# Distributed-Deep-Learning/ps

Measured on AMD Instinct MI355X. Metric: samples/sec (whole node) ResNet-50 sync-BSP at 1/2/4/8 MI355X workers, higher is better.
Workload: dtype bf16; 1 GPU; model=ResNet-50, global_batch=1024, image_size=224, parallelism=ps-bsp-colocated-dp1, optimizer=momentum@lr:0.1@momentum:0.9@wd:5e-05@nesterov:0.0@, staleness=0, fused_bn=True, ranks_per_device=1, compute_priority=high, side_stream=True, streams_per_rank=3, data_plane=local

## Files before the change

csrc/bindings.cpp:

```cpp
#include <torch/extension.h>
#include <c10/hip/HIPStream.h>
#include <c10/core/DeviceGuard.h>

#include "psamd_launch.h"

#include <atomic>
#include <map>
#include <mutex>
#include <string>

namespace {

std::atomic<bool> g_route_on{false};
std::mutex g_route_mu;
std::map<std::string, int64_t>& routes() {
  static std::map<std::string, int64_t> r;
  return r;
}
void route(const std::string& name) {
  if (!g_route_on.load(std::memory_order_relaxed)) return;
  std::lock_guard<std::mutex> g(g_route_mu);
  routes()[name] += 1;
}
std::map<std::string, int64_t> route_log(bool enable, bool reset) {
// ... 1693 lines not shown
                              want_mask ? mb.data_ptr<uint8_t>() : nullptr, R, static_cast<int>(C),
                              static_cast<int>(act), cur_stream(x));
  return {y, mb};
}

void weight_prep(Tensor jobs, int64_t max_blocks) {
  check_gpu(jobs, "jobs");
  TORCH_CHECK(jobs.scalar_type() == torch::kInt64 && jobs.dim() == 2 && jobs.size(1) == 4 && jobs.is_contiguous(),
              "jobs: int64 [J, 4]");
  static_assert(sizeof(void*) == 8, "64-bit pointers");
  const c10::DeviceGuard guard(jobs.device());
  TORCH_CHECK(max_blocks > 0 && max_blocks < (1 << 20), "max_blocks");
  psamd::launch_weight_prep(jobs.data_ptr(), static_cast<int>(jobs.size(0)), static_cast<int>(max_blocks),
                            cur_stream(jobs));
}

std::vector<Tensor> bn_bwd_coef(Tensor part, c10::optional<Tensor> gamma, Tensor mean, Tensor invstd, int64_t R) {
  check_part_slabs(part);
  const int64_t C = part.size(2);
  TORCH_CHECK(C % 8 == 0, "C % 8");
  const c10::DeviceGuard guard(part.device());
  auto fopt = part.options();
  auto dg = torch::empty({C}, fopt), db = torch::empty({C}, fopt), coef = torch::empty({3 * C}, fopt);
  const Tensor fp = fold_partials(part, cur_stream(part));
  const int64_t Gf = fp.size(1);
  psamd::launch_bn_bwd_partials(fp.data_ptr<float>(), fp.data_ptr<float>() + fp.stride(0), static_cast<int>(Gf), nullptr,
                                nullptr, f32_opt(gamma, C, "gamma"), f32_opt(mean, C, "mean"), f32_opt(invstd, C, "invstd"),
                                dg.data_ptr<float>(), db.data_ptr<float>(), coef.data_ptr<float>(), nullptr, R,
                                static_cast<int>(C), cur_stream(part));
  return {dg, db, coef};
}

std::vector<Tensor> bn_bwd_partials(Tensor g, Tensor x, Tensor part, c10::optional<Tensor> gamma, Tensor mean,
                                    Tensor invstd) {
  check_rows(g, "g");
  check_rows(x, "x");
  TORCH_CHECK(x.dim() == 2 && g.sizes() == x.sizes() && x.size(1) % 8 == 0, "g/x [R, C], C % 8");
  const int64_t R = x.size(0), C = x.size(1);
  check_part_slabs(part);
  TORCH_CHECK(part.size(2) == C, "part [2, G, C]");
  const c10::DeviceGuard guard(x.device());
  auto fopt = x.options().dtype(torch::kFloat32);
  auto dx = torch::empty_like(x);
  auto dg = torch::empty({C}, fopt), db = torch::empty({C}, fopt), coef = torch::empty({3 * C}, fopt);
  const Tensor fp = fold_partials(part, cur_stream(x));
  const int64_t Gf = fp.size(1);
  psamd::launch_bn_bwd_partials(fp.data_ptr<float>(), fp.data_ptr<float>() + fp.stride(0), static_cast<int>(Gf), u16(g), u16(x),
                                f32_opt(gamma, C, "gamma"), f32_opt(mean, C, "mean"), f32_opt(invstd, C, "invstd"),
                                dg.data_ptr<float>(), db.data_ptr<float>(), coef.data_ptr<float>(), u16m(dx), R,
                                static_cast<int>(C), cur_stream(x));
  return {dx, dg, db};
}

}

void register_async_ps(pybind11::module& m);
void register_plane(pybind11::module& m);
void register_async_rows(pybind11::module& m);

PYBIND11_MODULE(TORCH_EXTENSION_NAME, m) {
  m.doc() = "ps_amd HIP kernels for MI355X (gfx950)";
  register_async_ps(m);
  register_plane(m);
  register_async_rows(m);
  m.def("conv_gemm", &conv_gemm, py::arg("a"), py::arg("b"), py::arg("geo"), py::arg("pro") = py::none(),
        py::arg("epi") = 0, py::arg("aux") = py::none(), py::arg("kshift") = py::none(), py::arg("mc") = py::none(),
        py::arg("mean") = py::none(), py::arg("invstd") = py::none(), py::arg("bits") = py::none(),
        py::arg("aux2") = py::none(), py::arg("bits2") = py::none(), py::arg("a2") = py::none(),
        py::arg("bwd") = py::none(), py::arg("aux3") = py::none(), py::arg("mean2") = py::none(),
        py::arg("invstd2") = py::none(), py::arg("pro2") = py::none(), py::arg("aout") = py::none(),
        py::arg("abits") = py::none(), py::arg("tbuf") = py::none());
  m.def("route_log", &route_log, py::arg("enable") = true, py::arg("reset") = true);
  m.def("linear_wgrad_db", &linear_wgrad_db);
  m.def("bn_bwd_coef", &bn_bwd_coef);
  m.def("weight_prep", &weight_prep, py::arg("jobs"), py::arg("max_blocks") = 1024);
  m.def("conv_dgrad_s2", &conv_dgrad_s2, py::arg("dz"), py::arg("wph"), py::arg("H"), py::arg("W"),
        py::arg("epi") = 0, py::arg("z") = py::none(), py::arg("mc") = py::none(), py::arg("mean") = py::none(),
        py::arg("invstd") = py::none());
  m.def("conv_wgrad", &conv_wgrad, py::arg("dz"), py::arg("x"), py::arg("geo"), py::arg("pro") = py::none());
  m.def("conv_wgrad_patch_ok", &conv_wgrad_patch_ok, py::arg("geo"), py::arg("images"), py::arg("N"), py::arg("C"));
  {
    py::dict epi;
    epi["STORE"] = static_cast<int>(psamd::kEpiStore);
    epi["STATS"] = static_cast<int>(psamd::kEpiStats);
    epi["ADD"] = static_cast<int>(psamd::kEpiAdd);
    epi["MASK_SUMS"] = static_cast<int>(psamd::kEpiMaskSums);
    epi["ADD_S2"] = static_cast<int>(psamd::kEpiAddS2);
    epi["ADD_MASKED"] = static_cast<int>(psamd::kEpiAddMasked);
    epi["FOLD_ADD_MASKED"] = static_cast<int>(psamd::kEpiFoldAddMasked);
    epi["FOLD_ADD"] = static_cast<int>(psamd::kEpiFoldAdd);
    epi["FOLD_ADD_S2"] = static_cast<int>(psamd::kEpiFoldAddS2);
    epi["FOLD_ADD_MASKED_DS"] = static_cast<int>(psamd::kEpiFoldAddMaskedDs);
    m.attr("EPI") = epi;
  }
  m.attr("kTwosrcGldsMinNk") = psamd::kTwosrcGldsMinNk;
  m.def("conv_gemm_plan", &conv_gemm_plan, py::arg("M"), py::arg("N"), py::arg("C"), py::arg("geo"),
        py::arg("pro") = false, py::arg("epi") = 0, py::arg("src2") = 0);
  m.def("conv11_bwd_fused", &conv11_bwd_fused, py::arg("g"), py::arg("z3"), py::arg("cbwd"), py::arg("wt"), py::arg("z2"),
        py::arg("cf2") = py::none(), py::arg("mean2") = py::none(), py::arg("invstd2") = py::none());
  m.def("conv11_bwd_fused_supported", &conv11_bwd_fused_supported, py::arg("ci"), py::arg("co"),
        py::arg("plain") = false);
  m.def("bn_apply_coef", &bn_apply_coef, py::arg("x"), py::arg("coef"), py::arg("res") = py::none(),
        py::arg("rcoef") = py::none(), py::arg("act") = 1, py::arg("want_mask") = false);
  m.def("bn_bwd_partials", &bn_bwd_partials);
  m.def("fused_opt", &fused_opt);
  m.def("sparse_opt", &sparse_opt, py::arg("kind"), py::arg("table"), py::arg("st0"), py::arg("st1"),
        py::arg("rows"), py::arg("grad"), py::arg("rowwise"), py::arg("skip_zero"), py::arg("lr"), py::arg("beta1"),
        py::arg("beta2"), py::arg("eps"), py::arg("wd"), py::arg("momentum"), py::arg("dampening"),
        py::arg("nesterov"), py::arg("adamw"), py::arg("bc1"), py::arg("bc2"), py::arg("l1"), py::arg("l2"),
        py::arg("fbeta"), py::arg("ftrl_mode"), py::arg("gscale"), py::arg("perm") = py::none(), py::arg("ncount") = py::none());
  m.def("sumsq", &sumsq);
  m.def("clip_factor", &clip_factor);
  m.def("cast_", &cast_);
  m.def("axpy_", &axpy_);
  m.def("reduce_n", &reduce_n);
  m.def("lerp", &lerp);
  m.def("onebit_pack", &onebit_pack, py::arg("g"), py::arg("err"), py::arg("words"), py::arg("scales"),
        py::arg("mom") = py::none(), py::arg("beta1") = 0.0);
  m.def("onebit_momentum", &onebit_momentum);
  m.def("onebit_unpack_reduce", &onebit_unpack_reduce);
  m.def("gather_rows", &gather_rows);
  m.def("segment_reduce_rows", &segment_reduce_rows);
  m.def("bag_pool_fwd", &bag_pool_fwd);
  m.def("bag_pool_bwd", &bag_pool_bwd);
  m.def("scatter_add_rows", &scatter_add_rows);
  m.def("embedding_bag_fwd", &embedding_bag_fwd);
  m.def("sparse_lr_fwd", &sparse_lr_fwd);
  m.def("lazy_init_rows", &lazy_init_rows, py::arg("table"), py::arg("rows"), py::arg("flags"), py::arg("seed"),
        py::arg("row_base"), py::arg("lo"), py::arg("hi"), py::arg("keys") = py::none());
  m.def("hash_slots", &hash_slots);
  m.def("rehash_rows", &rehash_rows);
  m.def("unique_runs", &unique_runs);
  m.def("softmax_temp_fwd", &softmax_temp_fwd);
  m.def("softmax_temp_bwd", &softmax_temp_bwd);
  m.def("softmax_xent", &softmax_xent);
  m.def("bce", &bce);
  m.def("maxpool2d_fwd", &maxpool2d_fwd);
  m.def("maxpool2d_bwd", &maxpool2d_bwd);
  m.def("im2col", &im2col);
  m.def("col2im", &col2im);
  m.def("dropout", &dropout);
  m.def("uniform_init", &uniform_init);
  m.def("gemm_nt", &gemm_nt);
  m.def("fc_bwd", &fc_bwd, py::arg("dy"), py::arg("y"), py::arg("x"), py::arg("w"), py::arg("dw") = py::none(),
        py::arg("db") = py::none(), py::arg("dx") = py::none(), py::arg("act") = 0);
  m.def("fc_fwd_f32", &fc_fwd_f32);
  m.def("act_bwd", &act_bwd);
  m.def("bn_act_fwd", &bn_act_fwd);
  m.def("bn_stats", &bn_stats);
  m.def("maxpool_nhwc_fwd", &maxpool_nhwc_fwd);
  m.def("stem_conv_fwd", &stem_conv_fwd, py::arg("x"), py::arg("wp"), py::arg("kshift") = py::none());
  m.def("bn_finalize_sums", &bn_finalize_sums);
  m.def("stem_conv_wrw", &stem_conv_wrw);
  m.def("stem_bwd_fused", &stem_bwd_fused);
  m.def("dlrm_interact_fwd", &dlrm_interact_fwd);
  m.def("rmsnorm_fwd", &rmsnorm_fwd);
  m.def("rmsnorm_bwd", &rmsnorm_bwd);
// ... 27 lines not shown
```

csrc/include/psamd_launch.h:

```cpp
#pragma once
#include <hip/hip_runtime.h>
#include <stdint.h>

#include <stdexcept>
#include <string>

namespace psamd {

struct FusedOptArgs {
  int kind;
  float* w;
  float* st0;
  float* st1;
  const void* g;
  int g_bf16;
  void* wout;
  int wout_bf16;
  int64_t n;
  float lr, beta1, beta2, eps, wd, momentum, dampening;
  int nesterov, adamw;
  float bc1, bc2;
  float l1, l2, fbeta;
  int ftrl_mode;
  float gscale;
// ... 388 lines not shown
  const uint16_t* z2;
  const float* cf2;
  const float* mean2;
  const float* invstd2;
  uint16_t* gy;
  float* part;
  float* ws;
  uint16_t* dw;
  int M;
};
bool conv11_bwd_fused_ok(int CI, int CO);
bool conv11_bwd_plain_ok(int CI, int CO);
bool conv11_bwd_built(int CI, int CO);
int conv11_bwd_blocks(int M, int CI, int CO);
int64_t conv11_bwd_ws(int M, int CI, int CO);
void launch_conv11_bwd_fused(const Conv11BwdArgs& a, int CI, int CO, hipStream_t s);

struct ConvWgradArgs {
  const uint16_t* dz;
  const uint16_t* x;
  int M, N, K;
  ConvGeo g;
  const float* pro;
  float* ws;
  uint16_t* dw;
  float* db;
  float* dbws;
  FastDiv fd_ohw, fd_ow;
};
int conv_wgrad_splits(int M, int N, int K, int C, bool pro);
int64_t conv_wgrad_ws_geo(int M, int N, int K, const ConvGeo& g, bool pro);
bool conv_wgrad_is_wide(int M, int N, int K, int C, bool pro);
int64_t conv_wgrad_ws(int M, int N, int K, int C, bool pro);
void launch_attn_fwd(const uint16_t* qkv, uint16_t* out, float* lse, int B, int S, int H, float scale, float p,
                     uint64_t seed, hipStream_t s);
void launch_attn_bwd(const uint16_t* qkv, const uint16_t* out, const uint16_t* dout, const float* lse, uint16_t* dqkv,
                     int B, int S, int H, float scale, float p, uint64_t seed, hipStream_t s);
void launch_attn_dropout_mask(uint8_t* mask, int64_t n, float p, uint64_t seed, hipStream_t s);
void launch_xent_fwd(const uint16_t* x, const int64_t* lab, int64_t R, int V, int64_t ignore, float* lse, float* loss,
                     hipStream_t s);
void launch_xent_bwd(const uint16_t* x, const int64_t* lab, const float* lse, int64_t R, int V, int64_t ignore,
                     const float* go, const float* count, uint16_t* dx, hipStream_t s);
void launch_fa_fwd(const uint16_t* q, const uint16_t* k, const uint16_t* v, uint16_t* out, float* lse, int B, int S,
                   int H, int KV, float scale, hipStream_t s);
void launch_fa_bwd(const uint16_t* q, const uint16_t* k, const uint16_t* v, const uint16_t* out, const uint16_t* dout,
                   const float* lse, float* dsum, uint16_t* dq, uint16_t* dk, uint16_t* dv, int B, int S, int H,
                   int KV, float scale, hipStream_t s);
void launch_conv_wgrad(const ConvWgradArgs& a, hipStream_t s);
void launch_bn_apply_coef(const uint16_t* x, const uint16_t* res, const float* coef, const float* rcoef, uint16_t* y,
                          uint8_t* mbits, int64_t R, int C, int act, hipStream_t s);
void launch_bn_bwd_partials(const float* pd, const float* px, int G, const uint16_t* g, const uint16_t* x,
                            const float* gamma, const float* mean, const float* invstd, float* dgamma, float* dbeta,
                            float* coef, uint16_t* dx, int64_t R, int C, hipStream_t s);

}
```

csrc/kernels/bn_act.hip:

```cpp
#include <algorithm>
#include <cstdlib>
#include <utility>

#include "psamd_device.h"
#include "psamd_launch.h"

namespace psamd {

constexpr int kRedTpr = 32;

struct RedGeom {
  int tpr;
  int rows_it;
};

__host__ __device__ inline RedGeom red_geom(int C) {
  int tpr = C / 8;
  if (tpr > kRedTpr) tpr = kRedTpr;
  int p = 1;
  while (p < tpr) p <<= 1;
  return {p, 256 / p};
}

int bn_red_blocks(int64_t R, int C) {
// ... 562 lines not shown
  const int grid = apply_grid(nvec);
  const bool fixed = (static_cast<int64_t>(grid) * 256) % (C / 8) == 0;
  const bool mask = mbits != nullptr;
#define PSAMD_LAUNCH(K, ...) hipLaunchKernelGGL((K<__VA_ARGS__>), dim3(grid), dim3(256), 0, s, ARGS)
#define PSAMD_FM(K, ...)                                                            \
  if (fixed) {                                                                      \
    if (mask) { PSAMD_LAUNCH(K, __VA_ARGS__, true, true); }                         \
    else { PSAMD_LAUNCH(K, __VA_ARGS__, true, false); }                             \
  } else {                                                                          \
    if (mask) { PSAMD_LAUNCH(K, __VA_ARGS__, false, true); }                        \
    else { PSAMD_LAUNCH(K, __VA_ARGS__, false, false); }                            \
  }
  if (rcoef) {
#define ARGS x, res, coef, rcoef, y, nvec, C, mbits
    if (act == 1) { PSAMD_FM(bn_apply_dual_kernel, 1) }
    else { PSAMD_FM(bn_apply_dual_kernel, 0) }
#undef ARGS
  } else {
#define ARGS x, res, coef, coef + C, y, nvec, C, mbits
    if (res) {
      if (act == 1) { PSAMD_FM(bn_apply_kernel, true, 1) }
      else { PSAMD_FM(bn_apply_kernel, true, 0) }
    } else {
      if (act == 1) { PSAMD_FM(bn_apply_kernel, false, 1) }
      else { PSAMD_FM(bn_apply_kernel, false, 0) }
    }
#undef ARGS
  }
#undef PSAMD_FM
#undef PSAMD_LAUNCH
}

void launch_bn_bwd_partials(const float* pd, const float* px, int G, const uint16_t* g, const uint16_t* x,
                            const float* gamma, const float* mean, const float* invstd, float* dgamma, float* dbeta,
                            float* coef, uint16_t* dx, int64_t R, int C, hipStream_t s) {
  hipLaunchKernelGGL(bn_bwd_finalize_kernel, dim3(C / 8), dim3(fin_threads(G)), 0, s, pd, px, G, C, R, gamma, mean,
                     invstd, dgamma, dbeta, coef, coef + C, coef + 2 * C);
  const int64_t nvec = R * C / 8;
  if (nvec <= 0 || dx == nullptr) return;
  const int grid = apply_grid(nvec);
  const bool fixed = (static_cast<int64_t>(grid) * 256) % (C / 8) == 0;
  const uint16_t* none = nullptr;
  const float* nomc = nullptr;
  uint16_t* nodres = nullptr;
  const uint8_t* nobits = nullptr;
  if (fixed)
    hipLaunchKernelGGL((bn_bwd_apply_kernel<0, false, true>), dim3(grid), dim3(256), 0, s, g, none, x, nomc, coef,
                       coef + C, coef + 2 * C, dx, nodres, nvec, C, nobits);
  else
    hipLaunchKernelGGL((bn_bwd_apply_kernel<0, false, false>), dim3(grid), dim3(256), 0, s, g, none, x, nomc, coef,
                       coef + C, coef + 2 * C, dx, nodres, nvec, C, nobits);
}

}
```

ps_amd/knobs.py:

```python
from __future__ import annotations

import os
from typing import Dict, FrozenSet

ENV = "PS_AMD_DISABLE"

ROUTES: Dict[str, str] = {
    "fused_block": "bottlenecks module by module (nn.Conv2d on MIOpen + BatchNormAct2d)",
    "conv3x3": "fused blocks' 3x3 convolutions on MIOpen instead of the implicit-GEMM kernels",
    "block_out": "block outputs applied by their own pass, not in the next conv1's prologue",
    "fold_bn3": "bn3's backward reduce as its own pass, not in the consumer's conv1 data-gradient epilogue",
    "fold_bn_ds": "the downsample BN's backward reduce as its own pass (epilogue 8 instead of 9)",
    "conv3_bwd_fused": "conv3's data + weight gradient as two GEMMs (dz3 through HBM)",
    "ds_bwd_fused": "the downsample's data + weight gradient as apply pass + two GEMMs",
    "weight_prep": "backward weight layouts built per block instead of in one launch per forward",
    "pool_bn_bwd": "stem max-pool backward and BN backward as separate passes",
    "stem_bwd_fused": "stem weight gradient reading a materialised dz",
    "splitk_wgrad": "linear weight gradients on hipBLASLt instead of the split-K kernel",
    "linear_fork": "linear weight gradients on the compute stream",
    "fused_relu": "Linear + ReLU as separate ops",
    "ps_linear": "PS-owned linear weight gradients through autograd's ordinary accumulation",
    "fused_attn": "short-sequence attention on SDPA",
    "flash_attn": "causal GQA attention on SDPA",
    "fused_xent": "cross-entropy on fp32 logits through F.cross_entropy",
    "bag_pool": "multi-hot bags pooled by gather_rows -> weight multiply -> segment_reduce_rows ([nnz, dim] in HBM)",
}

_cache: Dict[str, FrozenSet[str]] = {}


def _parse(raw: str) -> FrozenSet[str]:
    got = _cache.get(raw)
    if got is None:
        got = frozenset(s.strip() for s in raw.split(",") if s.strip())
        bad = sorted(got - set(ROUTES))
        if bad:
            raise ValueError(f"{ENV}: unknown route(s) {bad}; known: {sorted(ROUTES)}")
        _cache[raw] = got
    return got


def disabled(route: str) -> bool:
    if route not in ROUTES:
        raise KeyError(f"unknown route {route!r}")
    raw = os.environ.get(ENV)
    return bool(raw) and route in _parse(raw)


def enabled(route: str) -> bool:
    return not disabled(route)
```

ps_amd/models/resnet.py:

```python
from __future__ import annotations


import torch
import torch.nn as nn

from .. import knobs
from ..ops.bn import BatchNormAct2d
from ..ops.conv import Conv1x1, StemConv, stem_bn_relu_maxpool
from ..ops.convgemm import (deferred_bn_counters, flush_deferred, fused_block_ok, fused_bottleneck,
                             prepare_backward_weights, resp_consumer_ok)
from ..ops.pool import MaxPool2d, global_avg_pool


class Bottleneck(nn.Module):
    expansion = 4

    def __init__(self, inplanes: int, planes: int, stride: int = 1, downsample: nn.Module | None = None,
                 fused_bn: bool = True):
        super().__init__()
        width = planes
        self.fused_bn = fused_bn
        BN = BatchNormAct2d if fused_bn else nn.BatchNorm2d
        C1 = Conv1x1 if fused_bn else (lambda i, o: nn.Conv2d(i, o, 1, bias=False))
        self.conv1 = C1(inplanes, width)
# ... 17 lines not shown
            return self.bn3(self.conv3(out), identity)
        out = self.relu(self.bn1(self.conv1(x)))
        out = self.relu(self.bn2(self.conv2(out)))
        out = self.bn3(self.conv3(out))
        return self.relu(out + identity)


class ResNet(nn.Module):
    def __init__(self, layers=(3, 4, 6, 3), num_classes: int = 1000, zero_init_residual: bool = True,
                 fused_bn: bool = True):
        super().__init__()
        self.inplanes = 64
        self.fused_bn = fused_bn
        self.conv1 = StemConv(3) if fused_bn else nn.Conv2d(3, 64, 7, stride=2, padding=3, bias=False)
        self.bn1 = BatchNormAct2d(64) if fused_bn else nn.BatchNorm2d(64)
        self.relu = nn.ReLU(inplace=True)
        self.maxpool = (MaxPool2d if fused_bn else nn.MaxPool2d)(3, stride=2, padding=1)
        self.layer1 = self._make_layer(64, layers[0])
        self.layer2 = self._make_layer(128, layers[1], stride=2)
        self.layer3 = self._make_layer(256, layers[2], stride=2)
        self.layer4 = self._make_layer(512, layers[3], stride=2)
        self.avgpool = nn.AdaptiveAvgPool2d((1, 1))
        self.fc = nn.Linear(512 * Bottleneck.expansion, num_classes)
        for m in self.modules():
            if isinstance(m, nn.Conv2d):
                nn.init.kaiming_normal_(m.weight, mode="fan_out", nonlinearity="relu")
            elif isinstance(m, nn.BatchNorm2d):
                nn.init.ones_(m.weight)
                nn.init.zeros_(m.bias)
        if zero_init_residual:
            for m in self.modules():
                if isinstance(m, Bottleneck):
                    nn.init.zeros_(m.bn3.weight)

    def _blocks(self):
        return [b for layer in (self.layer1, self.layer2, self.layer3, self.layer4) for b in layer]

    def _make_layer(self, planes: int, blocks: int, stride: int = 1) -> nn.Sequential:
        downsample = None
        if stride != 1 or self.inplanes != planes * 4:
            bn = BatchNormAct2d(planes * 4, act="none") if self.fused_bn else nn.BatchNorm2d(planes * 4)
            downsample = nn.Sequential(nn.Conv2d(self.inplanes, planes * 4, 1, stride=stride, bias=False), bn)
        layers = [Bottleneck(self.inplanes, planes, stride, downsample, self.fused_bn)]
        self.inplanes = planes * 4
        for _ in range(1, blocks):
            layers.append(Bottleneck(self.inplanes, planes, fused_bn=self.fused_bn))
        return nn.Sequential(*layers)

    def forward(self, x):
        if self.fused_bn:
            x = stem_bn_relu_maxpool(x, self.conv1, self.bn1)
        else:
            x = self.maxpool(self.relu(self.bn1(self.conv1(x))))
        with deferred_bn_counters():
            if self.fused_bn and self.training and x.is_cuda:
                blks = self._blocks()
                prepare_backward_weights(blks)
                on = knobs.enabled("block_out")
                h, w = x.shape[2], x.shape[3]
                for a, b in zip(blks, blks[1:] + [None]):
                    s = a.conv2.stride[0]
                    h, w = (h - 1) // s + 1, (w - 1) // s + 1
                    a._defer_out = (on and b is not None and b.fuse_block
                                    and resp_consumer_ok(b, x.shape[0] * h * w))
            x = self.layer4(self.layer3(self.layer2(self.layer1(x))))
        if self.fused_bn:
            x = global_avg_pool(x)
        else:
            x = torch.flatten(self.avgpool(x), 1)
        return self.fc(x)


def resnet50(num_classes: int = 1000, fused_bn: bool = True) -> ResNet:
    return ResNet((3, 4, 6, 3), num_classes, fused_bn=fused_bn)


def resnet_tiny(num_classes: int = 10, fused_bn: bool = True) -> ResNet:
    return ResNet((1, 1, 1, 1), num_classes, fused_bn=fused_bn)


def prepare_for_mi355x(model: nn.Module, dtype=torch.bfloat16, bn_fp32: bool = True) -> nn.Module:
    model = model.to(memory_format=torch.channels_last)
    for mod in model.modules():
        is_bn = isinstance(mod, nn.modules.batchnorm._BatchNorm)
        if is_bn and bn_fp32:
            continue
        for _, p in list(mod.named_parameters(recurse=False)):
            p.data = p.data.to(dtype)
        for name, b in list(mod.named_buffers(recurse=False)):
            if b.is_floating_point():
                setattr(mod, name, b.to(dtype))
    return model
```

ps_amd/ops/convgemm.py:

```python
from __future__ import annotations

import contextlib
import enum
import threading
import weakref
from typing import List

import torch
import torch.nn as nn
import torch.nn.functional as F

from .. import knobs
from . import side_stream as _side
from ._ext import native


def rows(x: torch.Tensor) -> torch.Tensor:
    n, c, h, w = x.shape
    if not x.is_contiguous(memory_format=torch.channels_last):
        x = x.contiguous(memory_format=torch.channels_last)
    return x.permute(0, 2, 3, 1).reshape(n * h * w, c)


def image(y2: torch.Tensor, n: int, h: int, w: int) -> torch.Tensor:
# ... 110 lines not shown
        self.z3, self.cf3, self.res, self.cfd, self.out, self.bits = z3, cf3, res, cfd, out, bits

    def flush(self) -> None:
        y, b = native().bn_apply_coef(self.z3, self.cf3, self.res, self.cfd, 1, True)
        with torch.no_grad():
            self.out.copy_(y)
            self.bits.copy_(b)


def _resp_enabled() -> bool:
    return knobs.enabled("block_out")


def big_tile(m: int, n: int, k: int, src2: int = Src2.NONE, epi: int = Epi.STATS, pro: bool = False) -> bool:
    return tuple(native().conv_gemm_plan(m, n, k, [m, 1, m, 1, 1, 1, 0], pro, int(epi), int(src2))[:2]) == (256, 256)


def resp_consumer_ok(blk: nn.Module, m: int = 0) -> bool:
    c1 = blk.conv1
    if m > 0 and big_tile(m, c1.out_channels, c1.in_channels, src2=Src2.BLOCK_OUT):
        return True
    return c1.out_channels <= TWOSRC_MAX_N and (
        c1.in_channels >= 64 * native().kTwosrcGldsMinNk or c1.out_channels <= 64)


def flush_deferred() -> None:
    pend = getattr(_tls, "pend", None)
    _tls.pend = None
    if pend is not None and pend.out_ref is not None and pend.out_ref() is not None:
        pend.flush()


def _bwd_prologue_enabled(n: int) -> bool:
    return n <= TWOSRC_MAX_N


def _conv3_bwd_fused(ci: int, co: int) -> bool:
    return knobs.enabled("conv3_bwd_fused") and bool(native().conv11_bwd_fused_supported(ci, co))


def _ds_bwd_fused(ci: int, co: int, s: int) -> bool:
    return (s == 1 and knobs.enabled("ds_bwd_fused")
            and bool(native().conv11_bwd_fused_supported(ci, co, True)))


def _fold_enabled() -> bool:
    return knobs.enabled("fold_bn3")


def _fold_ds_enabled() -> bool:
    return knobs.enabled("fold_bn_ds")


def _conv1_dgrad_epi(downsample: bool, stride: int, fold: bool, producer_ds: bool) -> Epi:
    if downsample:
        if stride == 2:
            return Epi.FOLD_ADD_S2 if fold else Epi.ADD_S2
        return Epi.FOLD_ADD if fold else Epi.ADD
    if not fold:
        return Epi.ADD_MASKED
    return Epi.FOLD_ADD_MASKED_DS if producer_ds else Epi.FOLD_ADD_MASKED


class _BottleneckFn(torch.autograd.Function):
    @staticmethod
    def forward(ctx, x, w1, g1, b1, w2, g2, b2, w3, g3, b3, wd, gd, bd, blk, link_in, pend_in):
        nat = native()
        n, cin, h, w = x.shape
        s = blk.conv2.stride[0]
        oh, ow = (h - 1) // s + 1, (w - 1) // s + 1
        gi, go = geo(h, w), geo(oh, ow)
        x2 = rows(x)
        bn1, bn2, bn3 = blk.bn1, blk.bn2, blk.bn3
        k1 = bn1.running_mean
        if pend_in is not None:
            z1, p1 = nat.conv_gemm(pend_in.z3, _mat(w1), gi, pro=pend_in.cf3, epi=Epi.STATS, kshift=k1,
                                   a2=pend_in.res, pro2=pend_in.cfd, aout=x2, abits=pend_in.bits)
            FOLD_STATS["resp"] += 1
        else:
            z1, p1 = nat.conv_gemm(x2, _mat(w1), gi, epi=Epi.STATS, kshift=k1)
        m1, i1, cf1 = _finalize(p1, k1, n * h * w, bn1)
        y1 = nat.bn_apply_coef(z1, cf1, None, None, 1)[0]
        if _conv3x3_enabled():
            k2 = bn2.running_mean
            z2r, p2s = nat.conv_gemm(y1, _mat3(w2), geo(h, w, 3, s, 1), epi=Epi.STATS, kshift=k2)
            m2, i2, cf2 = _finalize(p2s, k2, n * oh * ow, bn2)
        else:
            z2r = rows(F.conv2d(image(y1, n, h, w), w2, None, s, 1))
            m2, i2, cf2 = nat.bn_stats(z2r, g2, b2, bn2.running_mean, bn2.running_var, True, _momentum(bn2),
                                       float(bn2.eps))
        k3 = bn3.running_mean
        if z2r.shape[1] <= PRO_FUSE_MAX_K:
            z3, p3 = nat.conv_gemm(z2r, _mat(w3), go, pro=cf2, epi=Epi.STATS, kshift=k3)
        else:
            z3, p3 = nat.conv_gemm(nat.bn_apply_coef(z2r, cf2, None, None, 1)[0], _mat(w3), go, epi=Epi.STATS,
                                   kshift=k3)
        m3, i3, cf3 = _finalize(p3, k3, n * oh * ow, bn3)
        cfd = None
        if wd is not None:
            bnd = blk.downsample[1]
            kd = bnd.running_mean
            zd, pd = nat.conv_gemm(x2, _mat(wd), geo(h, w, 1, s), epi=Epi.STATS, kshift=kd)
            md, idd, cfd = _finalize(pd, kd, n * oh * ow, bnd)
        else:
            zd = md = idd = None
        if (getattr(blk, "_defer_out", False) and getattr(_tls, "pending", None) is not None
                and _resp_enabled()):
            out = torch.empty_like(z3)
            obits = torch.empty(z3.numel() // 8, dtype=torch.uint8, device=z3.device)
            _tls.pend_new = _Deferred(z3, cf3, zd if wd is not None else x2, cfd, out, obits)
        else:
            out, obits = nat.bn_apply_coef(z3, cf3, zd if wd is not None else x2, cfd, 1, True)
        ctx.save_for_backward(x2, w1, w2, w3, wd, g1, g2, g3, gd, z1, y1, z2r, z3, obits, zd,
                              m1, i1, cf1, m2, i2, cf2, m3, i3, md, idd)
        ctx.dims = (n, h, w, s, oh, ow)
        ctx.prep = _prep_for(blk, w1, w2, w3)
        ctx.link_in = link_in
        ctx.link_out = (_Link(z3, obits, m3, i3, zd if _fold_ds_enabled() else None, md, idd)
                        if _fold_enabled() else None)
        return image(out, n, oh, ow)

    @staticmethod
    def backward(ctx, dout):
        nat = native()
        (x2, w1, w2, w3, wd, g1, g2, g3, gd, z1, y1, z2r, z3, obits, zd,
         m1, i1, cf1, m2, i2, cf2, m3, i3, md, idd) = ctx.saved_tensors
        n, h, w, s, oh, ow = ctx.dims
        gi, go = geo(h, w), geo(oh, ow)
        d2 = rows(dout)
        sd = _side.Fork(d2.device, (w1, w2, w3, wd), images=n)
        pw = ctx.prep
        w3t = pw[1] if pw else _mat(w3).t()
        lk = ctx.link_out
        dz3 = dw3f = None
        ds_part = None
        if (lk is not None and lk.part is not None and d2.data_ptr() == lk.dx_ptr
                and d2._version == lk.dx_version):
            if lk.part.shape[0] == 3:
                ds_part = lk.part[0::2]
                lk.part = lk.part[:2]
                FOLD_STATS["ds"] += 1
            if (_bwd_prologue_enabled(w3.shape[1])
                    or big_tile(d2.shape[0], w3.shape[1], z3.shape[1], src2=Src2.BN_BWD, epi=Epi.MASK_SUMS)):
                dg3, db3, cb3 = nat.bn_bwd_coef(lk.part, g3, m3, i3, d2.shape[0])
                if _conv3_bwd_fused(w3.shape[1], w3.shape[0]):
                    gy2, p2, dw3f = nat.conv11_bwd_fused(d2, z3, cb3, w3t.contiguous(), z2r, cf2, m2, i2)
                    FOLD_STATS["conv3_fused"] = FOLD_STATS.get("conv3_fused", 0) + 1
                else:
                    gy2, p2, dz3 = nat.conv_gemm(d2, w3t, go, epi=Epi.MASK_SUMS, aux=z2r, mc=cf2, mean=m2, invstd=i2,
                                                 a2=z3, bwd=cb3)
            else:
                dz3, dg3, db3 = nat.bn_bwd_partials(d2, z3, lk.part, g3, m3, i3)
                gy2 = None
            FOLD_STATS["used"] += 1
        else:
            dz3, _, dg3, db3 = nat.bn_act_bwd(d2, None, z3, g3, m3, i3, 3, False, True, None, obits)
            gy2 = None
        if lk is not None:
            lk.part = lk.dx_keep = None
        if dw3f is not None:
            dw3 = _side._match_layout(dw3f, w3)
        else:
            sd.fork()
            dw3 = sd.run(lambda: nat.conv_wgrad(dz3, z2r, go, cf2), dz3, z2r, cf2, like=w3)
        if gy2 is None:
            gy2, p2 = nat.conv_gemm(dz3, w3t, go, epi=Epi.MASK_SUMS, aux=z2r, mc=cf2, mean=m2, invstd=i2)
        dz2, dg2, db2 = nat.bn_bwd_partials(gy2, z2r, p2, g2, m2, i2)
        c1, c2 = w2.shape[1], w2.shape[0]
        ours_dgrad = _conv3x3_enabled() and (s == 1 or (s == 2 and h % 2 == 0 and w % 2 == 0
                                                         and w2.shape[1] >= DGRAD_S2_MIN_C))
        ours_wgrad = _conv3x3_enabled() and (c1 >= WGRAD3X3_MIN_C
                                             or nat.conv_wgrad_patch_ok(geo(h, w, 3, s, 1), n, c2, c1))
        dy1 = dw2 = None
        sd.fork()
        if ours_wgrad:
            dw2 = sd.run(lambda: nat.conv_wgrad(dz2, y1, geo(h, w, 3, s, 1)).view(w2.shape[0], 3, 3, c1)
                         .permute(0, 3, 1, 2), dz2, y1, like=w2)
        else:
            dw2 = sd.run(lambda: torch.ops.aten.convolution_backward(
                image(dz2, n, oh, ow), image(y1, n, h, w), w2, None, [s, s], [1, 1], [1, 1], False, [0, 0], 1,
                [False, True, False])[1], dz2, y1, like=w2)
        if not ours_dgrad:
            dy1 = torch.ops.aten.convolution_backward(image(dz2, n, oh, ow), image(y1, n, h, w), w2, None,
                                                      [s, s], [1, 1], [1, 1], False, [0, 0], 1,
                                                      [True, False, False])[0]
        if ours_dgrad:
            if s == 1:
                gy1, p1b = nat.conv_gemm(dz2, pw[2] if pw else _mat3_dgrad(w2), geo(oh, ow, 3, 1, 1),
                                         epi=Epi.MASK_SUMS, aux=z1, mc=cf1, mean=m1, invstd=i1)
            else:
                gy1, p1b = nat.conv_dgrad_s2(dz2, pw[2] if pw else _phase_weights(w2), h, w, epi=Epi.MASK_SUMS, z=z1,
                                             mc=cf1, mean=m1, invstd=i1)
        li = ctx.link_in
        fold = li is not None and _fold_enabled()
        fkw = dict(mean=li.mean, invstd=li.invstd, aux2=li.z3, bits2=li.bits) if fold else {}
        e1 = _conv1_dgrad_epi(wd is not None, s, fold, fold and li.zd is not None)
        if e1 == Epi.FOLD_ADD_MASKED_DS:
            fkw.update(aux3=li.zd, mean2=li.md, invstd2=li.idd)
        if ours_dgrad:
            dz1, dg1, db1 = nat.bn_bwd_partials(gy1, z1, p1b, g1, m1, i1)
        else:
            dz1, _, dg1, db1 = nat.bn_act_bwd(rows(dy1), None, z1, g1, m1, i1, 1, False, True, cf1)
        sd.fork()
        dw1 = sd.run(lambda: nat.conv_wgrad(dz1, x2, gi), dz1, x2, like=w1)
        a1 = dz1
        w1t = pw[0] if pw else _mat(w1).t()
        dwd = dgd = dbd = None
        if wd is not None:
            wdt = pw[3] if pw else _mat(wd).t()
            if ds_part is not None and _ds_bwd_fused(wd.shape[1], wd.shape[0], s):
                dgd, dbd, cbd = nat.bn_bwd_coef(ds_part, gd, md, idd, d2.shape[0])
                t, _, dwdf = nat.conv11_bwd_fused(d2, zd, cbd, wdt.contiguous(), x2)
                dwd = _side._match_layout(dwdf, wd)
                FOLD_STATS["ds_fused"] = FOLD_STATS.get("ds_fused", 0) + 1
            else:
                if ds_part is not None:
                    dzd, dgd, dbd = nat.bn_bwd_partials(d2, zd, ds_part, gd, md, idd)
                else:
                    dzd, _, dgd, dbd = nat.bn_act_bwd(d2, None, zd, gd, md, idd, 3, False, True, None, obits)
                sd.fork()
                dwd = sd.run(lambda: nat.conv_wgrad(dzd, x2, geo(h, w, 1, s)), dzd, x2, like=wd)
                t = nat.conv_gemm(dzd, wdt, go, epi=Epi.STORE)[0]
            r1 = nat.conv_gemm(a1, w1t, gi, epi=e1, aux=t, **fkw)
        else:
            r1 = nat.conv_gemm(a1, w1t, gi, epi=e1, aux=d2, bits=obits, **fkw)
        dx2, part = r1[0], r1[1]
        if fold:
            li.part, li.dx_ptr, li.dx_version, li.dx_keep = part, dx2.data_ptr(), dx2._version, dx2
        return (image(dx2, n, h, w), dw1, dg1, db1, dw2, dg2, db2, dw3, dg3, db3,
                dwd, dgd, dbd, None, None, None)


def fused_block_ok(blk: nn.Module, x: torch.Tensor) -> bool:
    if knobs.disabled("fused_block") or not getattr(blk, "fuse_block", False):
        return False
    if not (blk.training and x.is_cuda and x.dtype == torch.bfloat16 and x.dim() == 4):
        return False
    ds = blk.downsample
    bns = [blk.bn1, blk.bn2, blk.bn3] + ([ds[1]] if ds is not None else [])
    for bn in bns:
        if not (bn.track_running_stats and bn.affine and bn.weight.dtype == torch.float32
                and bn.running_mean is not None and bn.running_mean.dtype == torch.float32):
            return False
    c1, c2, c3 = blk.conv1, blk.conv2, blk.conv3
    convs = [c1, c2, c3] + ([ds[0]] if ds is not None else [])
    if any(not isinstance(c, nn.Conv2d) or c.weight.dtype != torch.bfloat16 or c.bias is not None or c.groups != 1
           for c in convs):
        return False
    if c1.kernel_size != (1, 1) or c1.stride != (1, 1) or c3.kernel_size != (1, 1) or c3.stride != (1, 1):
        return False
    if (c2.kernel_size != (3, 3) or c2.padding != (1, 1) or c2.dilation != (1, 1)
            or c2.stride[0] != c2.stride[1] or c2.stride[0] not in (1, 2)):
        return False
    if ds is not None:
        if len(ds) != 2 or ds[0].kernel_size != (1, 1) or ds[0].stride != c2.stride or ds[0].padding != (0, 0):
            return False
        if getattr(ds[1], "act", "none") != "none":
            return False
    elif c2.stride != (1, 1) or x.shape[1] != c3.out_channels:
        return False
    return all(c % 64 == 0 for c in (x.shape[1], c1.out_channels, c3.out_channels))


_tls = threading.local()

_PREP_CACHE: "dict" = {}


def _prep_ok(blk: nn.Module) -> bool:
    ws = [blk.conv1.weight, blk.conv2.weight, blk.conv3.weight] + (
        [blk.downsample[0].weight] if blk.downsample is not None else [])
    return (getattr(blk, "fuse_block", False) and all(w.is_cuda and w.dtype == torch.bfloat16 for w in ws)
            and blk.conv2.weight.is_contiguous(memory_format=torch.channels_last)
            and all(w.is_contiguous() for w in [blk.conv1.weight, blk.conv3.weight] + ws[3:]))


def prepare_backward_weights(blocks) -> None:
    if knobs.disabled("weight_prep"):
# ... 105 lines not shown
```

Baseline: 16710 samples/s.

## Fuse last block's bn3+residual+ReLU with global average pooling

For the final bottleneck block, the forward now applies bn3, adds the residual, applies ReLU and average-pools in one kernel. It writes only the pooled [N, C] output and a ReLU bitmask instead of the full activation. Backward expands the pooled gradient on the fly in two new kernels, one for the BN statistics and one that emits dz3 and the residual gradient. This removes a full-size activation write and read plus the separate pool passes, at the cost of new code paths and special-casing in the block backward.

```diff
diff --git a/csrc/bindings.cpp b/csrc/bindings.cpp
--- a/csrc/bindings.cpp
+++ b/csrc/bindings.cpp
@@ -1769,6 +1769,63 @@
   return {dx, dg, db};
 }
 
+static int64_t pool_tail_images(const Tensor& z, int64_t hw, const char* name) {
+  check_rows(z, name);
+  TORCH_CHECK(z.dim() == 2 && z.size(1) % 8 == 0 && hw > 0 && hw < (1 << 20) && z.size(0) % hw == 0 && z.size(0) > 0,
+              name, " [N * hw, C], C % 8");
+  return z.size(0) / hw;
+}
+static void pool_tail_check(const Tensor& gp, const Tensor& bits, const Tensor& z, int64_t N) {
+  check_rows(gp, "gp");
+  TORCH_CHECK(gp.dim() == 2 && gp.size(0) == N && gp.size(1) == z.size(1), "gp [N, C]");
+  check_gpu(bits, "bits");
+  TORCH_CHECK(bits.scalar_type() == torch::kUInt8 && bits.is_contiguous() && bits.numel() == z.numel() / 8,
+              "bits: uint8 [N * hw * C / 8]");
+}
+
+std::vector<Tensor> pool_tail_fwd(Tensor z, Tensor coef, Tensor res, int64_t hw) {
+  const int64_t N = pool_tail_images(z, hw, "z"), C = z.size(1);
+  check_rows(res, "res");
+  TORCH_CHECK(res.sizes() == z.sizes(), "res like z");
+  check_f32(coef, "coef");
+  TORCH_CHECK(coef.numel() == 2 * C && coef.is_contiguous(), "coef = [scale | shift]");
+  const c10::DeviceGuard guard(z.device());
+  auto pooled = torch::empty({N, C}, z.options());
+  auto mb = torch::empty({z.numel() / 8}, z.options().dtype(torch::kUInt8));
+  route("pool_tail/fwd");
+  psamd::launch_pool_tail_fwd(u16(z), u16(res), coef.data_ptr<float>(), N, static_cast<int>(hw), static_cast<int>(C),
+                              u16m(pooled), mb.data_ptr<uint8_t>(), cur_stream(z));
+  return {pooled, mb};
+}
+
+Tensor pool_tail_bwd_stats(Tensor gp, Tensor bits, Tensor z, Tensor mean, Tensor invstd, int64_t hw) {
+  const int64_t N = pool_tail_images(z, hw, "z"), C = z.size(1);
+  pool_tail_check(gp, bits, z, N);
+  const float* mu = f32_opt(mean, C, "mean");
+  const float* is = f32_opt(invstd, C, "invstd");
+  TORCH_CHECK(mu && is, "mean, invstd [C]");
+  const c10::DeviceGuard guard(z.device());
+  const int G = psamd::pool_tail_blocks(N, static_cast<int>(C));
+  auto part = torch::empty({2, G, C}, z.options().dtype(torch::kFloat32));
+  route("pool_tail/bwd_stats");
+  psamd::launch_pool_tail_bwd_stats(u16(gp), bits.data_ptr<uint8_t>(), u16(z), mu, is, N, static_cast<int>(hw),
+                                    static_cast<int>(C), part.data_ptr<float>(), cur_stream(z));
+  return part;
+}
+
+std::vector<Tensor> pool_tail_bwd_apply(Tensor gp, Tensor bits, Tensor z, Tensor coef, int64_t hw) {
+  const int64_t N = pool_tail_images(z, hw, "z"), C = z.size(1);
+  pool_tail_check(gp, bits, z, N);
+  check_f32(coef, "coef");
+  TORCH_CHECK(coef.numel() == 3 * C && coef.is_contiguous(), "coef = [ca | cb | cc]");
+  const c10::DeviceGuard guard(z.device());
+  auto dz = torch::empty_like(z), dres = torch::empty_like(z);
+  route("pool_tail/bwd_apply");
+  psamd::launch_pool_tail_bwd_apply(u16(gp), bits.data_ptr<uint8_t>(), u16(z), coef.data_ptr<float>(), N,
+                                    static_cast<int>(hw), static_cast<int>(C), u16m(dz), u16m(dres), cur_stream(z));
+  return {dz, dres};
+}
+
 }
 
 void register_async_ps(pybind11::module& m);
@@ -1820,6 +1877,11 @@
   m.def("bn_apply_coef", &bn_apply_coef, py::arg("x"), py::arg("coef"), py::arg("res") = py::none(),
         py::arg("rcoef") = py::none(), py::arg("act") = 1, py::arg("want_mask") = false);
   m.def("bn_bwd_partials", &bn_bwd_partials);
+  m.def("pool_tail_fwd", &pool_tail_fwd, py::arg("z"), py::arg("coef"), py::arg("res"), py::arg("hw"));
+  m.def("pool_tail_bwd_stats", &pool_tail_bwd_stats, py::arg("gp"), py::arg("bits"), py::arg("z"), py::arg("mean"),
+        py::arg("invstd"), py::arg("hw"));
+  m.def("pool_tail_bwd_apply", &pool_tail_bwd_apply, py::arg("gp"), py::arg("bits"), py::arg("z"), py::arg("coef"),
+        py::arg("hw"));
   m.def("fused_opt", &fused_opt);
   m.def("sparse_opt", &sparse_opt, py::arg("kind"), py::arg("table"), py::arg("st0"), py::arg("st1"),
         py::arg("rows"), py::arg("grad"), py::arg("rowwise"), py::arg("skip_zero"), py::arg("lr"), py::arg("beta1"),
diff --git a/csrc/include/psamd_launch.h b/csrc/include/psamd_launch.h
--- a/csrc/include/psamd_launch.h
+++ b/csrc/include/psamd_launch.h
@@ -464,5 +464,12 @@
 void launch_bn_bwd_partials(const float* pd, const float* px, int G, const uint16_t* g, const uint16_t* x,
                             const float* gamma, const float* mean, const float* invstd, float* dgamma, float* dbeta,
                             float* coef, uint16_t* dx, int64_t R, int C, hipStream_t s);
-
-}
+void launch_pool_tail_fwd(const uint16_t* z, const uint16_t* res, const float* coef, int64_t N, int HW, int C,
+                          uint16_t* pooled, uint8_t* mbits, hipStream_t s);
+int pool_tail_blocks(int64_t N, int C);
+void launch_pool_tail_bwd_stats(const uint16_t* gp, const uint8_t* mbits, const uint16_t* z, const float* mean,
+                                const float* invstd, int64_t N, int HW, int C, float* part, hipStream_t s);
+void launch_pool_tail_bwd_apply(const uint16_t* gp, const uint8_t* mbits, const uint16_t* z, const float* coef,
+                                int64_t N, int HW, int C, uint16_t* dz, uint16_t* dres, hipStream_t s);
+
+}
diff --git a/csrc/kernels/bn_act.hip b/csrc/kernels/bn_act.hip
--- a/csrc/kernels/bn_act.hip
+++ b/csrc/kernels/bn_act.hip
@@ -638,4 +638,216 @@
                        coef + C, coef + 2 * C, dx, nodres, nvec, C, nobits);
 }
 
-}
+constexpr int kPoolU = 7;
+
+__global__ __launch_bounds__(256) void pool_tail_fwd_kernel(const uint16_t* __restrict__ z,
+                                                            const uint16_t* __restrict__ res,
+                                                            const float* __restrict__ scale,
+                                                            const float* __restrict__ shift, int64_t nthr, int HW,
+                                                            int C, float inv_hw, uint16_t* __restrict__ pooled,
+                                                            uint8_t* __restrict__ mb) {
+  const int64_t t = static_cast<int64_t>(blockIdx.x) * blockDim.x + threadIdx.x;
+  if (t >= nthr) return;
+  const int cvec = C / 8;
+  const int64_t n = t / cvec;
+  const int cg = static_cast<int>(t - n * cvec);
+  float sc[8], sh[8], acc[8] = {0, 0, 0, 0, 0, 0, 0, 0};
+  load8(scale, cg * 8, sc);
+  load8(shift, cg * 8, sh);
+  auto one = [&](int64_t v, float (&a)[8], const float (&b)[8]) {
+    unsigned bits = 0;
+#pragma unroll
+    for (int j = 0; j < 8; ++j) {
+      float o = a[j] * sc[j] + sh[j];
+      o += b[j];
+      o = o > 0.f ? o : 0.f;
+      bits |= (o > 0.f ? 1u : 0u) << j;
+      acc[j] += bf16_to_f32(f32_to_bf16(o));
+    }
+    mb[v] = static_cast<uint8_t>(bits);
+  };
+  int64_t v = n * HW * cvec + cg;
+  int p = 0;
+  for (; p + kPoolU <= HW; p += kPoolU, v += static_cast<int64_t>(kPoolU) * cvec) {
+    float a[kPoolU][8], b[kPoolU][8];
+#pragma unroll
+    for (int u = 0; u < kPoolU; ++u) {
+      load8(z, (v + static_cast<int64_t>(u) * cvec) * 8, a[u]);
+      load8(res, (v + static_cast<int64_t>(u) * cvec) * 8, b[u]);
+    }
+#pragma unroll
+    for (int u = 0; u < kPoolU; ++u) one(v + static_cast<int64_t>(u) * cvec, a[u], b[u]);
+  }
+  for (; p < HW; ++p, v += cvec) {
+    float a[8], b[8];
+    load8(z, v * 8, a);
+    load8(res, v * 8, b);
+    one(v, a, b);
+  }
+#pragma unroll
+  for (int j = 0; j < 8; ++j) acc[j] *= inv_hw;
+  store8(pooled, t * 8, acc);
+}
+
+__device__ __forceinline__ void pool_grad8(const uint16_t* __restrict__ gp, int64_t i, float inv_hw, float (&g)[8]) {
+  load8(gp, i, g);
+#pragma unroll
+  for (int j = 0; j < 8; ++j) g[j] = bf16_to_f32(f32_to_bf16(g[j] * inv_hw));
+}
+
+inline int pool_tail_ipb(int64_t N, int C) {
+  const int slots = red_geom(C).rows_it;
+  const int64_t g = std::min<int64_t>((N + slots - 1) / slots, 2048);
+  return static_cast<int>((N + g - 1) / g);
+}
+int pool_tail_blocks(int64_t N, int C) {
+  const int ipb = pool_tail_ipb(N, C);
+  return static_cast<int>((N + ipb - 1) / ipb);
+}
+
+__global__ __launch_bounds__(256) void pool_tail_bwd_stats_kernel(const uint16_t* __restrict__ gp,
+                                                                  const uint8_t* __restrict__ mb,
+                                                                  const uint16_t* __restrict__ z,
+                                                                  const float* __restrict__ mean,
+                                                                  const float* __restrict__ invstd, int64_t N,
+                                                                  int HW, int C, int ipb, float inv_hw,
+                                                                  float* __restrict__ pd, float* __restrict__ px) {
+  __shared__ float lds_d[256 * 8];
+  __shared__ float lds_x[256 * 8];
+  const RedGeom gm = red_geom(C);
+  const int t = threadIdx.x;
+  const int cg = t % gm.tpr + blockIdx.y * kRedTpr;
+  const int slot = t / gm.tpr;
+  const int cvec = C / 8;
+  const int64_t nb = static_cast<int64_t>(blockIdx.x) * ipb;
+  const int64_t ne = nb + ipb < N ? nb + ipb : N;
+  float sd[8] = {0, 0, 0, 0, 0, 0, 0, 0}, sx[8] = {0, 0, 0, 0, 0, 0, 0, 0};
+  if (cg < cvec) {
+    float mu[8], is[8];
+    load8(mean, cg * 8, mu);
+    load8(invstd, cg * 8, is);
+    for (int64_t n = nb + slot; n < ne; n += gm.rows_it) {
+      float g[8];
+      pool_grad8(gp, (n * cvec + cg) * 8, inv_hw, g);
+      auto acc = [&](const float (&xv)[8], unsigned bits) {
+#pragma unroll
+        for (int j = 0; j < 8; ++j) {
+          const float gj = (bits >> j) & 1u ? g[j] : 0.f;
+          sd[j] += gj;
+          sx[j] += gj * (xv[j] - mu[j]) * is[j];
+        }
+      };
+      int64_t v = n * HW * cvec + cg;
+      int p = 0;
+      for (; p + kPoolU <= HW; p += kPoolU, v += static_cast<int64_t>(kPoolU) * cvec) {
+        float xv[kPoolU][8];
+        unsigned bits[kPoolU];
+#pragma unroll
+        for (int u = 0; u < kPoolU; ++u) {
+          load8(z, (v + static_cast<int64_t>(u) * cvec) * 8, xv[u]);
+          bits[u] = mb[v + static_cast<int64_t>(u) * cvec];
+        }
+#pragma unroll
+        for (int u = 0; u < kPoolU; ++u) acc(xv[u], bits[u]);
+      }
+      for (; p < HW; ++p, v += cvec) {
+        float xv[8];
+        load8(z, v * 8, xv);
+        acc(xv, mb[v]);
+      }
+    }
+  }
+#pragma unroll
+  for (int j = 0; j < 8; ++j) {
+    lds_d[t * 8 + j] = sd[j];
+    lds_x[t * 8 + j] = sx[j];
+  }
+  __syncthreads();
+  if (slot == 0 && cg < cvec) {
+    for (int k = 1; k < gm.rows_it; ++k) {
+      const int src = (k * gm.tpr + t) * 8;
+#pragma unroll
+      for (int j = 0; j < 8; ++j) {
+        sd[j] += lds_d[src + j];
+        sx[j] += lds_x[src + j];
+      }
+    }
+    store8(pd, blockIdx.x * static_cast<int64_t>(C) + cg * 8, sd);
+    store8(px, blockIdx.x * static_cast<int64_t>(C) + cg * 8, sx);
+  }
+}
+
+__global__ __launch_bounds__(256) void pool_tail_bwd_apply_kernel(const uint16_t* __restrict__ gp,
+                                                                  const uint8_t* __restrict__ mb,
+                                                                  const uint16_t* __restrict__ z,
+                                                                  const float* __restrict__ ca,
+                                                                  const float* __restrict__ cb,
+                                                                  const float* __restrict__ cc, int64_t nthr, int HW,
+                                                                  int C, float inv_hw, uint16_t* __restrict__ dz,
+                                                                  uint16_t* __restrict__ dres) {
+  const int64_t t = static_cast<int64_t>(blockIdx.x) * blockDim.x + threadIdx.x;
+  if (t >= nthr) return;
+  const int cvec = C / 8;
+  const int64_t n = t / cvec;
+  const int cg = static_cast<int>(t - n * cvec);
+  float A[8], B[8], Cc[8], g[8];
+  load8(ca, cg * 8, A);
+  load8(cb, cg * 8, B);
+  load8(cc, cg * 8, Cc);
+  pool_grad8(gp, t * 8, inv_hw, g);
+  auto one = [&](int64_t v, float (&xv)[8], unsigned bits) {
+    float gm[8];
+#pragma unroll
+    for (int j = 0; j < 8; ++j) gm[j] = (bits >> j) & 1u ? g[j] : 0.f;
+    store8(dres, v * 8, gm);
+#pragma unroll
+    for (int j = 0; j < 8; ++j) xv[j] = A[j] * gm[j] + B[j] * xv[j] + Cc[j];
+    store8(dz, v * 8, xv);
+  };
+  int64_t v = n * HW * cvec + cg;
+  int p = 0;
+  for (; p + kPoolU <= HW; p += kPoolU, v += static_cast<int64_t>(kPoolU) * cvec) {
+    float xv[kPoolU][8];
+    unsigned bits[kPoolU];
+#pragma unroll
+    for (int u = 0; u < kPoolU; ++u) {
+      load8(z, (v + static_cast<int64_t>(u) * cvec) * 8, xv[u]);
+      bits[u] = mb[v + static_cast<int64_t>(u) * cvec];
+    }
+#pragma unroll
+    for (int u = 0; u < kPoolU; ++u) one(v + static_cast<int64_t>(u) * cvec, xv[u], bits[u]);
+  }
+  for (; p < HW; ++p, v += cvec) {
+    float xv[8];
+    load8(z, v * 8, xv);
+    one(v, xv, mb[v]);
+  }
+}
+
+inline int pool_tail_grid(int64_t nthr) { return static_cast<int>((nthr + 255) / 256); }
+
+void launch_pool_tail_fwd(const uint16_t* z, const uint16_t* res, const float* coef, int64_t N, int HW, int C,
+                          uint16_t* pooled, uint8_t* mbits, hipStream_t s) {
+  const int64_t nthr = N * (C / 8);
+  if (nthr <= 0) return;
+  hipLaunchKernelGGL(pool_tail_fwd_kernel, dim3(pool_tail_grid(nthr)), dim3(256), 0, s, z, res, coef, coef + C, nthr,
+                     HW, C, static_cast<float>(1.0 / HW), pooled, mbits);
+}
+
+void launch_pool_tail_bwd_stats(const uint16_t* gp, const uint8_t* mbits, const uint16_t* z, const float* mean,
+                                const float* invstd, int64_t N, int HW, int C, float* part, hipStream_t s) {
+  const int G = pool_tail_blocks(N, C);
+  const int ctiles = (C / 8 + kRedTpr - 1) / kRedTpr;
+  hipLaunchKernelGGL(pool_tail_bwd_stats_kernel, dim3(G, ctiles), dim3(256), 0, s, gp, mbits, z, mean, invstd, N, HW,
+                     C, pool_tail_ipb(N, C), static_cast<float>(1.0 / HW), part, part + static_cast<int64_t>(G) * C);
+}
+
+void launch_pool_tail_bwd_apply(const uint16_t* gp, const uint8_t* mbits, const uint16_t* z, const float* coef,
+                                int64_t N, int HW, int C, uint16_t* dz, uint16_t* dres, hipStream_t s) {
+  const int64_t nthr = N * (C / 8);
+  if (nthr <= 0) return;
+  hipLaunchKernelGGL(pool_tail_bwd_apply_kernel, dim3(pool_tail_grid(nthr)), dim3(256), 0, s, gp, mbits, z, coef,
+                     coef + C, coef + 2 * C, nthr, HW, C, static_cast<float>(1.0 / HW), dz, dres);
+}
+
+}
diff --git a/ps_amd/knobs.py b/ps_amd/knobs.py
--- a/ps_amd/knobs.py
+++ b/ps_amd/knobs.py
@@ -13,6 +13,7 @@
     "fold_bn_ds": "the downsample BN's backward reduce as its own pass (epilogue 8 instead of 9)",
     "conv3_bwd_fused": "conv3's data + weight gradient as two GEMMs (dz3 through HBM)",
     "ds_bwd_fused": "the downsample's data + weight gradient as apply pass + two GEMMs",
+    "pool_tail": "the last block's output stored and pooled by global_avg_pool, its bn3 backward from the expanded gradient",
     "weight_prep": "backward weight layouts built per block instead of in one launch per forward",
     "pool_bn_bwd": "stem max-pool backward and BN backward as separate passes",
     "stem_bwd_fused": "stem weight gradient reading a materialised dz",
diff --git a/ps_amd/models/resnet.py b/ps_amd/models/resnet.py
--- a/ps_amd/models/resnet.py
+++ b/ps_amd/models/resnet.py
@@ -93,9 +93,12 @@
             x = stem_bn_relu_maxpool(x, self.conv1, self.bn1)
         else:
             x = self.maxpool(self.relu(self.bn1(self.conv1(x))))
+        last = None
         with deferred_bn_counters():
             if self.fused_bn and self.training and x.is_cuda:
                 blks = self._blocks()
+                last = blks[-1]
+                last._pool_out = True
                 prepare_backward_weights(blks)
                 on = knobs.enabled("block_out")
                 h, w = x.shape[2], x.shape[3]
@@ -104,8 +107,14 @@
                     h, w = (h - 1) // s + 1, (w - 1) // s + 1
                     a._defer_out = (on and b is not None and b.fuse_block
                                     and resp_consumer_ok(b, x.shape[0] * h * w))
-            x = self.layer4(self.layer3(self.layer2(self.layer1(x))))
-        if self.fused_bn:
+            try:
+                x = self.layer4(self.layer3(self.layer2(self.layer1(x))))
+            finally:
+                if last is not None:
+                    last._pool_out = False
+        if x.dim() == 2:
+            pass
+        elif self.fused_bn:
             x = global_avg_pool(x)
         else:
             x = torch.flatten(self.avgpool(x), 1)
diff --git a/ps_amd/ops/convgemm.py b/ps_amd/ops/convgemm.py
--- a/ps_amd/ops/convgemm.py
+++ b/ps_amd/ops/convgemm.py
@@ -186,6 +186,10 @@
     return knobs.enabled("fold_bn_ds")
 
 
+def pool_tail_ok(blk: nn.Module) -> bool:
+    return bool(getattr(blk, "_pool_out", False)) and blk.downsample is None and knobs.enabled("pool_tail")
+
+
 def _conv1_dgrad_epi(downsample: bool, stride: int, fold: bool, producer_ds: bool) -> Epi:
     if downsample:
         if stride == 2:
@@ -238,7 +242,10 @@
             md, idd, cfd = _finalize(pd, kd, n * oh * ow, bnd)
         else:
             zd = md = idd = None
-        if (getattr(blk, "_defer_out", False) and getattr(_tls, "pending", None) is not None
+        ctx.pooled = pool_tail_ok(blk)
+        if ctx.pooled:
+            out, obits = nat.pool_tail_fwd(z3, cf3, x2, oh * ow)
+        elif (getattr(blk, "_defer_out", False) and getattr(_tls, "pending", None) is not None
                 and _resp_enabled()):
             out = torch.empty_like(z3)
             obits = torch.empty(z3.numel() // 8, dtype=torch.uint8, device=z3.device)
@@ -251,8 +258,8 @@
         ctx.prep = _prep_for(blk, w1, w2, w3)
         ctx.link_in = link_in
         ctx.link_out = (_Link(z3, obits, m3, i3, zd if _fold_ds_enabled() else None, md, idd)
-                        if _fold_enabled() else None)
-        return image(out, n, oh, ow)
+                        if _fold_enabled() and not ctx.pooled else None)
+        return out if ctx.pooled else image(out, n, oh, ow)
 
     @staticmethod
     def backward(ctx, dout):
@@ -261,14 +268,20 @@
          m1, i1, cf1, m2, i2, cf2, m3, i3, md, idd) = ctx.saved_tensors
         n, h, w, s, oh, ow = ctx.dims
         gi, go = geo(h, w), geo(oh, ow)
-        d2 = rows(dout)
-        sd = _side.Fork(d2.device, (w1, w2, w3, wd), images=n)
+        d2 = None if ctx.pooled else rows(dout)
+        sd = _side.Fork(dout.device, (w1, w2, w3, wd), images=n)
         pw = ctx.prep
         w3t = pw[1] if pw else _mat(w3).t()
         lk = ctx.link_out
         dz3 = dw3f = None
         ds_part = None
-        if (lk is not None and lk.part is not None and d2.data_ptr() == lk.dx_ptr
+        if ctx.pooled:
+            gp = dout.contiguous()
+            part3 = nat.pool_tail_bwd_stats(gp, obits, z3, m3, i3, oh * ow)
+            dg3, db3, cb3 = nat.bn_bwd_coef(part3, g3, m3, i3, z3.shape[0])
+            dz3, d2 = nat.pool_tail_bwd_apply(gp, obits, z3, cb3, oh * ow)
+            gy2 = None
+        elif (lk is not None and lk.part is not None and d2.data_ptr() == lk.dx_ptr
                 and d2._version == lk.dx_version):
             if lk.part.shape[0] == 3:
                 ds_part = lk.part[0::2]
@@ -328,7 +341,7 @@
         li = ctx.link_in
         fold = li is not None and _fold_enabled()
         fkw = dict(mean=li.mean, invstd=li.invstd, aux2=li.z3, bits2=li.bits) if fold else {}
-        e1 = _conv1_dgrad_epi(wd is not None, s, fold, fold and li.zd is not None)
+        e1 = _conv1_dgrad_epi(wd is not None or ctx.pooled, s, fold, fold and li.zd is not None)
         if e1 == Epi.FOLD_ADD_MASKED_DS:
             fkw.update(aux3=li.zd, mean2=li.md, invstd2=li.idd)
         if ours_dgrad:
@@ -357,7 +370,7 @@
                 t = nat.conv_gemm(dzd, wdt, go, epi=Epi.STORE)[0]
             r1 = nat.conv_gemm(a1, w1t, gi, epi=e1, aux=t, **fkw)
         else:
-            r1 = nat.conv_gemm(a1, w1t, gi, epi=e1, aux=d2, bits=obits, **fkw)
+            r1 = nat.conv_gemm(a1, w1t, gi, epi=e1, aux=d2, bits=None if ctx.pooled else obits, **fkw)
         dx2, part = r1[0], r1[1]
         if fold:
             li.part, li.dx_ptr, li.dx_version, li.dx_keep = part, dx2.data_ptr(), dx2._version, dx2
```

Result: no change. 16800 samples/s, median of 6 (+0.5%).
